# zhexin1904/gtsam_personal

Measured on AMD Instinct MI355X. Metric: LM iterations/sec, higher is better.
Workload: dtype f64; 1 GPU; synthetic BAL 1000 cameras / 100000 points / 1000002 factors (GeneralSFMFactor<Cal3Bundler> + 2 priors), seed 42, METIS ordering (Ordering::Metis of the reference, fixture-carried permutation), LM legacy defaults; ordering=metis, cameras=1000, points=100000, factors=1000002, fronts=100001, parallelism=single GPU

## Files before the change

### gtsam_personal_amd/csrc/kernels_dense.hpp

```cpp
#pragma once
#include <hip/hip_runtime.h>

#include <type_traits>
#include <vector>

#include "kernels_front.hpp"

namespace lmgpu {

typedef double double4_t __attribute__((ext_vector_type(4)));

struct RowSrc {
  int32_t idx;
  int32_t i;
};
inline int32_t append_row_sources(const FrontDesc& F, const std::vector<ChildRef>& childs, const std::vector<int32_t>& cmap, const std::vector<FrontFac>& ffac,
                                  const std::vector<FacDesc>& fd, std::vector<int32_t>& rowptr, std::vector<RowSrc>& rowsrc) {
  std::vector<std::vector<RowSrc>> rows(F.n);
  for (int k = 0; k < F.child_count; k++) {
    const ChildRef& c = childs[F.child_begin + k];
    for (int i = 0; i < c.m; i++) rows[cmap[c.map_begin + i]].push_back(RowSrc{F.child_begin + k, i});
  }
  for (int k = 0; k < F.fac_count; k++) {
    const FrontFac& ff = ffac[F.fac_begin + k];
// ... 35 lines not shown
      const double* J = pool + d.joff;
      const int m = d.rows, nc = d.d0 + d.d1 + d.d2 + 1, p = sr.i;
      for (int q = lane; q < nc; q += 64) {
        const int gq = fac_col(d, ff.c0, ff.c1, ff.c2, q, F.n);
        if (gq > R || (gq == R && q == p)) {
          double v = 0;
          for (int r = 0; r < m; r++) v += J[p * m + r] * J[q * m + r];
          Arow[gq] += v;
        }
      }
    }
    __builtin_amdgcn_fence(__ATOMIC_RELEASE, "wavefront");
    asm volatile("s_waitcnt vmcnt(0)" ::: "memory");
    __builtin_amdgcn_fence(__ATOMIC_ACQUIRE, "wavefront");
  }
}
__global__ __launch_bounds__(256) void hbm_assemble_rows_kernel(FrontDesc F, int64_t f_off, int ld, const int32_t* __restrict__ rowptr,
                                                                const RowSrc* __restrict__ src, const ChildRef* __restrict__ childs,
                                                                const int32_t* __restrict__ cmap, const FrontFac* __restrict__ ffac,
                                                                const FacDesc* __restrict__ fd, double* __restrict__ pool, int with_factors) {
  const int R = blockIdx.x * 4 + (threadIdx.x >> 6);
  if (R >= F.n) return;
  assemble_row_body(F, f_off, ld, rowptr, src, childs, cmap, ffac, fd, pool, R, with_factors != 0);
}

__global__ __launch_bounds__(256) void hbm_damp_kernel(FrontDesc F, int64_t f_off, int ld, const int32_t* __restrict__ fxoff,
                                                        double* __restrict__ pool, double lambda_v, const double* __restrict__ lambda_p, const double* __restrict__ dampw,
                                                        const double* __restrict__ gex) {
  const int i = blockIdx.x * 256 + threadIdx.x;
  if (i >= F.nf) return;
  pool[f_off + (size_t)i * ld + i] += (lambda_p ? *lambda_p : lambda_v) * dampw[fxoff[F.fx_begin + i]];
  if (gex) pool[f_off + (size_t)i * ld + F.n - 1] += gex[fxoff[F.fx_begin + i]];
}

struct ZeroRange {
  int64_t off, count;
};
__global__ __launch_bounds__(256) void zero_ranges_kernel(const ZeroRange* __restrict__ ranges, double* __restrict__ pool) {
  const ZeroRange r = ranges[blockIdx.y];
  double2* p = (double2*)(pool + r.off);
  const int64_t n2 = r.count >> 1;
  for (int64_t i = (int64_t)blockIdx.x * 256 + threadIdx.x; i < n2; i += (int64_t)gridDim.x * 256) p[i] = double2{0.0, 0.0};
}

#define FILL_CHUNK_BYTES 32768
struct FillChunk {
// ... 934 lines not shown
```

### gtsam_personal_amd/csrc/kernels_potrf.hpp

```cpp
#pragma once
#include <hip/hip_runtime.h>

namespace lmgpu {

typedef double double4_t __attribute__((ext_vector_type(4)));

__device__ __forceinline__ double readlane_d(double v, int src_lane) {
  const long long b = __double_as_longlong(v);
  const int lo = __builtin_amdgcn_readlane((int)(b & 0xffffffffLL), src_lane);
  const int hi = __builtin_amdgcn_readlane((int)(b >> 32), src_lane);
  return __longlong_as_double(((long long)hi << 32) | (unsigned int)lo);
}

__device__ __forceinline__ double fast_rsqrt(double p) {
  double y = __builtin_amdgcn_rsq(p);
  const double h = 0.5 * p;
  y = y * fma(-h * y, y, 1.5);
  y = y * fma(-h * y, y, 1.5);
  return y;
}

template <bool INV>
__device__ __forceinline__ bool potrf64_wave_g4(double4_t (&T)[4][4], double4_t (&E)[4], int nrows = 64) {
  const int lane = threadIdx.x & 63, kk = lane >> 4, cc = lane & 15;
// ... 293 lines not shown
          }
        double4_t out = double4_t{0, 0, 0, 0};
#pragma unroll
        for (int sx = 0; sx < 4; sx++) out = __builtin_amdgcn_mfma_f64_16x16x4f64(I16[4 * j + g][4 * sx + kk][cc], acc[sx], out, 0, 0, 0);
        T[g] = out;
        X[j][g] = out;
#pragma unroll
        for (int r = 0; r < 4; r++) {
          const int row = 16 * g + kk + 4 * r;
          if (row < nbj && cvalid) P[(size_t)(64 * j + row) * ld + c0 + cc] = out[r];
        }
      }
    }
  }
}

__global__ __launch_bounds__(256) void panel_trsm_kernel(double* __restrict__ A, int ld, int n, int ko, int kb, const double* __restrict__ inv16) {
  __shared__ double I16[16][16][17];
  panel_trsm_body(A, ld, n, ko, kb, inv16, I16, blockIdx.x);
}

#define TAIL_MAX_M 48
#define TAIL_MAX_KP 256
#define TAIL_LDS_BYTES ((TAIL_MAX_KP * TAIL_MAX_M + TAIL_MAX_M * TAIL_MAX_M + 64 * 65) * 8)
__global__ __launch_bounds__(256) void front_tail_kernel(double* __restrict__ A, int ld, int n, int nf, int p0, int kp, int front_id,
                                                         int* __restrict__ status, double* __restrict__ inv16) {
  extern __shared__ double tsm[];
  const int r0 = p0 + kp, m = n - r0, nft = nf - r0, tid = threadIdx.x;
  double* Pl = tsm;
  double* S = tsm + (size_t)TAIL_MAX_KP * TAIL_MAX_M;
  double(*D)[65] = (double(*)[65])(S + TAIL_MAX_M * TAIL_MAX_M);
  for (int idx = tid; idx < kp * m; idx += 256) {
    const int k = idx / m, j = idx - k * m;
    Pl[idx] = A[(size_t)(p0 + k) * ld + r0 + j];
  }
  for (int idx = tid; idx < m * m; idx += 256) {
    const int i = idx / m, j = idx - i * m;
    S[idx] = (j >= i) ? A[(size_t)(r0 + i) * ld + r0 + j] : 0.0;
  }
  __syncthreads();
  for (int idx = tid; idx < m * m; idx += 256) {
    const int i = idx / m, j = idx - i * m;
    if (j < i) continue;
    double s0 = 0.0, s1 = 0.0;
    int k = 0;
    for (; k + 1 < kp; k += 2) {
      s0 += Pl[k * m + i] * Pl[k * m + j];
      s1 += Pl[(k + 1) * m + i] * Pl[(k + 1) * m + j];
    }
// ... 34 lines not shown
  for (int idx = tid; idx < m * m; idx += 256) {
    const int i = idx / m, j = idx - i * m;
    if (j >= i) A[(size_t)(r0 + i) * ld + r0 + j] = S[idx];
  }
  for (int idx = tid; idx < 64 * 64; idx += 256) {
    const int p = idx >> 6, q = idx & 63;
    D[p][q] = (p < nft && q < nft && q >= p) ? S[p * m + q] : ((p == q) ? 1.0 : 0.0);
  }
  __syncthreads();
  if (tid < 64) {
    const int blk = tid >> 4, c = tid & 15, base = 16 * blk;
    double x[16];
#pragma unroll
    for (int i = 15; i >= 0; i--) {
      double sacc = (i == c) ? 1.0 : 0.0;
#pragma unroll
      for (int kq = i + 1; kq < 16; kq++) sacc -= D[base + i][base + kq] * x[kq];
      x[i] = (i <= c) ? sacc / D[base + i][base + i] : 0.0;
    }
#pragma unroll
    for (int i = 0; i < 16; i++) inv16[(size_t)blk * 256 + i * 16 + c] = x[i];
  }
}

#ifndef PDF_STAMP
#define PDF_STAMP(flags, b, slot)
#endif
#define PDF_TA0 32
#define PDF_MAX_COLTILES 992
#define PDF_PR0 1024
#define PDF_TD0 1536
#define PDF_FLAG_WORDS 8192
#define PDF_MAX_CHAIN_T 114
#define PDF_SPIN_LIMIT 2000000L
#define PDF_LDS_DOUBLES (2 * 64 * DP_LDW)
#define PDF_LDS_BYTES (PDF_LDS_DOUBLES * 8)

__host__ __device__ inline unsigned int pdf_ta_need(int sj) { return sj < 4 ? 4u * (unsigned int)(sj + 1) : 2u; }

__device__ __forceinline__ bool pdf_wait(unsigned int* flags, int w0, unsigned int need0, int w1, unsigned int need1, int* s_ok, int tid) {
  if (tid == 0) {
    bool ok = true;
    for (int q = 0; q < 2 && ok; q++) {
      const int w = q ? w1 : w0;
      const unsigned int need = q ? need1 : need0;
      if (w < 0) continue;
// ... 256 lines not shown
```

### gtsam_personal_amd/csrc/lmgpu.hip

```cpp
#include <hip/hip_runtime.h>
#include <rccl/rccl.h>

#include <algorithm>
#include <chrono>
#include <cmath>
#include <cstdio>
#include <cstdlib>
#include <cstring>
#include <condition_variable>
#include <limits>
#include <mutex>
#include <string>
#include <map>
#include <vector>

#include "../../include/lmgpu.h"
#include "kernels_dense.hpp"
#include "kernels_potrf.hpp"
#include "kernels_step.hpp"
#include "dense_schedule.hpp"
#include "dogleg_step.hpp"
#include "kernels_batched.hpp"
#include "kernels_level.hpp"
#include "kernels_bayes.hpp"
// ... 217 lines not shown
  };
  std::vector<ElimSeg> elim_segs;
  std::vector<int> elim_seg_of;
  bool merge_elim = false;
  FillUpper* d_fill_upper = nullptr;
  int n_fill_upper = 0;
  bool fuse_levels = false;
  LevelTask* d_level_tasks = nullptr;
  LevelSync* d_level_sync = nullptr;
  int n_level_sync = 0;
  int32_t *d_bs_parent = nullptr, *d_bs_pos = nullptr;
  char* d_leafpack = nullptr;
  unsigned int* d_bs_done = nullptr;
  bool use_graph = false;
  int eager_solves = 0;
  hipGraphExec_t solve_graph[2] = {nullptr, nullptr};
  int leaf_group_threads = 256;
  bool no_backsub_groups = false;
  int n_leaf_group_launches = 0;
  bool no_wide16 = false;
  int wide16_max = 256;
  bool bsd_ticket = false;
  bool no_tail = false;
  bool no_chain = false;
  int chain_forms = 0;
  unsigned int* d_pflags = nullptr;
  int pflags_panels = 0;
  unsigned int* bs_flags = nullptr;
  double* pool = nullptr;
  size_t pool_doubles = 0;
  double* vals[2][kNumVarTypes] = {};
  double* saved[kNumVarTypes] = {};
  int cur = 0;
  int32_t* type_xoff[kNumVarTypes] = {};
  double *delta = nullptr, *dampw = nullptr, *hdiag = nullptr, *ebuf0 = nullptr, *ebuf1 = nullptr, *partial = nullptr, *dscal = nullptr,
         *ywork = nullptr;
  int* d_status = nullptr;
  double* h_scal = nullptr;
  int* h_status = nullptr;
  FacDesc* d_fd = nullptr;
  FrontDesc* d_fronts = nullptr;
  FrontFac* d_ffac = nullptr;
  ChildRef* d_childs = nullptr;
  int32_t *d_cmap = nullptr, *d_fxoff = nullptr, *d_sxoff = nullptr, *d_lists = nullptr;
  int32_t *d_hbm_small = nullptr, *d_f_ld = nullptr, *d_med_list = nullptr;
  MedFront* d_med_fronts = nullptr;
  BsdBlock* d_bsd_table = nullptr;
  struct BsdRun {
    int lvl_hi, lvl_lo, begin, count;
  };
  std::vector<BsdRun> bsd_runs;
// ... 323 lines not shown
      h->dampw_is_ones = true;
    }
    return LMGPU_OK;
  }
  int rc = launch_hessian_diag(h);
  if (rc) return rc;
  hipLaunchKernelGGL(clamp_diag_kernel, dim3((h->ntot + 255) / 256), dim3(256), 0, h->stream, h->ntot, (const double*)h->hdiag, h->dampw, min_diag, max_diag);
  h->dampw_is_ones = false;
  return LMGPU_OK;
}

static bool gather_writes(const lmgpu_handle* h, int fi) {
  const lmgpu_handle::GatherRange& G = h->gather[fi];
  if (!(G.write_ok && G.leaf_count > 0 && !h->no_gather_write && h->n_hbm_fronts <= 4)) return false;
  if (h->s_off[fi] < 0) return true;
  return (h->h_fronts[fi].pad & 1) != 0 && (h->comm || h->lgroup);
}

static void add_fill(std::vector<FillChunk>& t, const void* p, size_t bytes, uint32_t value) {
  for (size_t o = 0; o < bytes; o += FILL_CHUNK_BYTES)
    t.push_back(FillChunk{(unsigned long long)(uintptr_t)p + o, (uint32_t)std::min<size_t>(FILL_CHUNK_BYTES, bytes - o), value});
}

static void launch_assemble_rows(lmgpu_handle* h, int fi, int64_t aoff, bool with_factors) {
  const FrontDesc& F = h->h_fronts[fi];
  if (h->row_begin[fi] >= 0 && (F.child_count > 0 || (with_factors && F.fac_count > 0)))
    hipLaunchKernelGGL(hbm_assemble_rows_kernel, dim3((F.n + 3) / 4), dim3(256), 0, h->stream, F, aoff, h->f_ld[fi], (const int32_t*)(h->d_rowptr + h->row_begin[fi]),
                       (const RowSrc*)h->d_rowsrc, (const ChildRef*)h->d_childs, (const int32_t*)h->d_cmap, (const FrontFac*)h->d_ffac,
                       (const FacDesc*)h->d_fd, h->pool, with_factors ? 1 : 0);
}

static void launch_hbm_damp(lmgpu_handle* h, int fi, int64_t aoff, double lambda_v, const double* lambda_p) {
  const FrontDesc& F = h->h_fronts[fi];
  hipLaunchKernelGGL(hbm_damp_kernel, dim3((F.nf + 255) / 256), dim3(256), 0, h->stream, F, aoff, h->f_ld[fi], (const int32_t*)h->d_fxoff, h->pool, lambda_v,
                     lambda_p, (const double*)h->dampw, (const double*)h->gex_active);
}

static int dense_mode_of(const lmgpu_handle* h, int fi) {
  const bool replicated = (h->h_fronts[fi].pad & 1) != 0;
  if (h->s_off[fi] < 0 || !replicated || !(h->comm || h->lgroup)) return DENSE_SINGLE;
  return h->comm ? DENSE_SPLIT_EVENTS : DENSE_SPLIT_HOST;
}

static void chunk_range(int n, int ld, int c, size_t& begin, size_t& count) {
  const int r0c = c * NBO, rows = std::min(n, r0c + NBO) - r0c;
  begin = (size_t)r0c * ld + r0c;
  count = (size_t)rows * ld - r0c;
}

static int wait_chunk(lmgpu_handle* h, double* Asm, int n, int ld, int c) {
  if (h->comm) {
    HIPCHECK(hipStreamWaitEvent(h->stream, h->chunk_ev[c], 0));
// ... 68 lines not shown
      lo = std::min(lo, h->f_off[fi]);
      hi = std::max(hi, h->f_off[fi] + cnt);
    }
  *lo_out = lo;
  *hi_out = hi;
  return n_hbm <= 4 ? HBM_CLEAR_EACH : (hi - lo <= 2 * sum ? HBM_CLEAR_SPAN : HBM_CLEAR_RANGES);
}

static bool backsub_merged(const lmgpu_handle* h) {
  return h->merge_backsub && h->cfg.world_size == 1 && !(h->cfg.flags & LMGPU_FLAG_SPLIT_ROOT);
}

static int ensure_fill_tables(lmgpu_handle* h) {
  int64_t lo, hi;
  const int regime = hbm_clear_regime(h, &lo, &hi);
  if (h->n_fill_elim < 0) {
    std::vector<FillChunk> fills;
    add_fill(fills, h->d_status, sizeof(int), 0x7f7f7f7fu);
    add_fill(fills, h->d_status + 1, sizeof(int), 0u);
    if (h->merge_elim || h->fuse_levels)
      add_fill(fills, h->d_bs_done, (size_t)(h->h_fronts.size() + h->levels.size() + 1) * sizeof(unsigned int), 0u);
    if (h->fuse_levels) add_fill(fills, h->d_level_sync, (size_t)h->n_level_sync * sizeof(LevelSync), 0u);
    if (regime == HBM_CLEAR_SPAN) add_fill(fills, h->pool + lo, (size_t)(hi - lo) * sizeof(double), 0u);
    h->n_fill_elim = (int)fills.size();
    const int rcu = upload(h, &h->d_fill_elim, fills);
    if (rcu) return rcu;
  }
  if (regime == HBM_CLEAR_RANGES && !h->d_zero_ranges) {
    std::vector<ZeroRange> zr;
    for (const LevelWork& L : h->levels)
      for (int fi : L.hbm) {
        const bool gw = gather_writes(h, fi);
        const int64_t cnt = (int64_t)h->h_fronts[fi].n * h->f_ld[fi];
        if (!gw || h->s_off[fi] >= 0) zr.push_back(ZeroRange{h->f_off[fi], cnt});
        if (!gw && h->s_off[fi] >= 0) zr.push_back(ZeroRange{h->s_off[fi], cnt});
      }
    h->n_zero_ranges = (int)zr.size();
    const int rcu = upload(h, &h->d_zero_ranges, zr);
    if (rcu) return rcu;
  }
  if (h->n_fill_backsub < 0) {
    std::vector<FillChunk> fills;
    if (backsub_merged(h)) {
      add_fill(fills, h->d_bs_done, (size_t)(h->h_fronts.size() + h->levels.size() + 1) * sizeof(unsigned int), 0u);
      add_fill(fills, h->delta, h->ntot * sizeof(double), 0xffffffffu);
    }
// ... 117 lines not shown
        ktm = h->kt.begin(LMGPU_KT_SYRK, s);
        hipLaunchKernelGGL(med_syrk_kernel, dim3(4 * S, S, cnt), dim3(256), 0, s, ML, h->pool);
        h->kt.end(ktm, s);
      }
    }
    for (int fi : L.hbm) {
      if (h->is_med[fi]) continue;
      const FrontDesc& F = h->h_fronts[fi];
      const int64_t off = h->f_off[fi];
      const int ld = h->f_ld[fi];
      double* A = h->pool + off;
      const bool own_terms = (F.pad & 2) == 0;
      const lmgpu_handle::GatherRange& G = h->gather[fi];
      const int nchunks = (F.n + NBO - 1) / NBO;
      const int mode = dense_mode_of(h, fi);
      const bool split = mode != DENSE_SINGLE;
      const int64_t aoff = split ? h->s_off[fi] : off;
      double* Asm = h->pool + aoff;

      const int kt = h->kt.begin(LMGPU_KT_HBM_ASSEMBLE, s);
      const bool gwrite = gather_writes(h, fi);
      if (gwrite && G.zero_count > 0)
        hipLaunchKernelGGL(zero_blocks_kernel, dim3(G.zero_count), dim3(128), 0, s, (const GZeroBlock*)(h->d_gzero + G.zero_begin), h->pool, aoff, ld);
      launch_assemble_rows(h, fi, aoff, own_terms && !gwrite);
      if (!gwrite && own_terms) launch_hbm_damp(h, fi, aoff, lambda_v, lambda_p);
      const int schur_masked = dev_switch("LMGPU_SCHUR_UNMASKED") ? 0 : 2;
      if (G.pblk_short > 0)
        hipLaunchKernelGGL((schur_pairs_kernel<1>), dim3((G.pblk_short + 7) & ~7), dim3(64), 0, s, (const GPairBlock*)(h->d_gpblk + G.pblk_begin),
                           (const GPairEntry*)h->d_gpent, h->pool, aoff, ld, G.pblk_short, (gwrite ? 1 : 0) | schur_masked);
      if (G.pblk_long > 0)
        hipLaunchKernelGGL((schur_pairs_kernel<4>), dim3((G.pblk_long + 7) & ~7), dim3(256), 0, s,
                           (const GPairBlock*)(h->d_gpblk + G.pblk_begin + G.pblk_short), (const GPairEntry*)h->d_gpent, h->pool, aoff, ld,
                           G.pblk_long, (gwrite ? 1 : 0) | schur_masked);
#ifdef LMGPU_TEST_HOOKS
      if (h->schur_split_diag) {
        if (G.vblk_count > 0)
          hipLaunchKernelGGL(schur_factor_kernel, dim3(G.vblk_count), dim3(64 * SCHUR_FW), 0, s, (const GVarBlock*)(h->d_gvblk + G.vblk_begin),
                             (const GVarEntry*)h->d_gvent, h->pool, aoff, ld, F.n, schur_masked);
        if (G.leaf_count > 0) {
          double* scal = h->dscal + 4;
          reduce_to(h, h->d_gcorner + G.leaf_begin, G.leaf_count, scal, s, nullptr);
          hipLaunchKernelGGL(add_scalar_kernel, dim3(1), dim3(1), 0, s, Asm + (size_t)(F.n - 1) * ld + F.n - 1, (const double*)scal);
        }
      } else
#endif
      {
        const int vlong = G.vblk_count - G.vblk_short;
        const int corner_short = (G.leaf_count > 0 && vlong == 0) ? 1 : 0, corner_long = (G.leaf_count > 0 && vlong > 0) ? 1 : 0;
        if (G.vblk_short + corner_short > 0)
          hipLaunchKernelGGL((schur_var_kernel<1>), dim3(G.vblk_short + corner_short), dim3(64), 0, s, (const GVarBlock*)(h->d_gvblk + G.vblk_begin),
                             (const GVarEntry*)h->d_gvent, h->pool, aoff, ld, F.n, G.vblk_short, gwrite ? 1 : 0,
                             (const double*)(h->d_gcorner + G.leaf_begin), G.leaf_count);
        if (vlong + corner_long > 0)
          hipLaunchKernelGGL((schur_var_kernel<SCHUR_VAR_WAVES>), dim3(vlong + corner_long), dim3(64 * SCHUR_VAR_WAVES), 0, s,
                             (const GVarBlock*)(h->d_gvblk + G.vblk_begin + G.vblk_short), (const GVarEntry*)h->d_gvent, h->pool, aoff, ld, F.n, vlong,
                             gwrite ? 1 : 0, (const double*)(h->d_gcorner + G.leaf_begin), G.leaf_count);
      }
      if (gwrite && own_terms) {
        if (F.fac_count > 0) launch_assemble_rows(h, fi, aoff, true);
        launch_hbm_damp(h, fi, aoff, lambda_v, lambda_p);
      }
      h->kt.end(kt, s);
      if (mode == DENSE_SPLIT_EVENTS) {
        HIPCHECK(hipEventRecord(h->asm_ev, s));
        HIPCHECK(hipStreamWaitEvent(h->comm_stream, h->asm_ev, 0));
        for (int c = 0; c < nchunks; c++) {
          size_t cb, cn;
          chunk_range(F.n, ld, c, cb, cn);
          NCCLCHECK(ncclAllReduce(Asm + cb, Asm + cb, cn, ncclDouble, ncclSum, h->comm_data ? h->comm_data : h->comm, h->comm_stream));
          HIPCHECK(hipEventRecord(h->chunk_ev[c], h->comm_stream));
        }
      }

      const lmgpu_handle::DensePlan& plan = h->dense_plans[fi];
      h->inv16_owner = fi;
      int kt_run = -1, run_launches = 0;
      double run_flop = 0;
      for (size_t r = 0; r < plan.steps.size(); r++) {
        const DenseStep& st = plan.steps[r];
        const int i = st.i, k0 = i * NBO, kb = std::min(F.nf, k0 + NBO) - k0, r0 = k0 + kb, m = F.n - r0;
        const bool in_run = st.kind == DENSE_STEP_FUSED || (st.kind == DENSE_WAIT_CHUNK && plan.steps[r + 1].kind == DENSE_STEP_FUSED);
        if (!in_run && run_launches > 0) {
          h->kt.end(kt_run, s, run_flop, run_launches);
          run_launches = 0;
          run_flop = 0;
        }
        switch (st.kind) {
          case DENSE_PANEL_DATAFLOW:
          case DENSE_PANEL_TWO_LAUNCH: {
            if (i == 0) HIPCHECK(hipMemsetAsync(h->d_pflags, 0, (size_t)((F.nf + NBO - 1) / NBO + 1) * PDF_FLAG_WORDS * sizeof(unsigned int), s));
            double* inv16 = h->inv16 + (size_t)i * 4096;
            const int ktp = h->kt.begin(LMGPU_KT_PANEL, s);
            if (st.kind == DENSE_PANEL_DATAFLOW) {
              hipLaunchKernelGGL(panel_dataflow_kernel, dim3(kb / 64 + (m + 63) / 64), dim3(256), PDF_LDS_BYTES, s, A, ld, F.n, F.nf, k0, kb, F.id,
                                 h->d_status, inv16, h->d_pflags + (size_t)i * PDF_FLAG_WORDS);
            } else {
              hipLaunchKernelGGL(diag_potrf_kernel, dim3(1), dim3(256), DIAG_LDS_BYTES, s, A, ld, F.nf, k0, kb, F.id, h->d_status, inv16);
              if (m > 0) hipLaunchKernelGGL(panel_trsm_kernel, dim3((m + 63) / 64), dim3(256), 0, s, A, ld, F.n, k0, kb, (const double*)inv16);
            }
            h->kt.end(ktp, s, st.flop);
            break;
          }
          case DENSE_CHAIN: {
            ChainArgs ca{A, ld, F.n, F.nf, i, st.nsteps, F.id, h->d_status, h->inv16, h->d_pflags, h->d_chain_tasks + plan.task_begin[r],
                         split ? (const double*)Asm : nullptr};
#ifdef LMGPU_TEST_HOOKS
            ca.dev_forms = h->chain_forms;
#endif
            const int ktc = h->kt.begin(LMGPU_KT_CHAIN, s);
            hipLaunchKernelGGL(chain_kernel, dim3(plan.task_count[r]), dim3(256), STEP_LDS_BYTES, s, ca);
            h->kt.end(ktc, s, st.flop, 1);
            break;
          }
// ... 5 lines not shown
            a.dev_forms = h->chain_forms;
#endif
            if (run_launches == 0) kt_run = h->kt.begin(LMGPU_KT_SYRK, s);
            hipLaunchKernelGGL(step_kernel, dim3(step_grid(m, kbn)), dim3(256), STEP_LDS_BYTES, s, a);
            run_launches++;
            run_flop += st.flop;
            break;
          }
          case DENSE_UPDATE_QUADRANTS:
          case DENSE_UPDATE_MFMA: {
            const int kts = h->kt.begin(LMGPU_KT_SYRK, s);
            if (st.kind == DENSE_UPDATE_QUADRANTS) {
              const int S = (m + 63) / 64;
              hipLaunchKernelGGL(syrk_quadrants_kernel, dim3(4 * S, S), dim3(256), 0, s, A, ld, F.n, k0, kb, r0);
            } else {
              const int T = (m + 127) / 128;
              hipLaunchKernelGGL(syrk_mfma_kernel, dim3(T, T), dim3(256), kSyrkLds, s, A, ld, F.n, k0, kb, r0, F.n);
            }
            h->kt.end(kts, s, st.flop);
            break;
          }
          case DENSE_TAIL: {
            const int ktt = h->kt.begin(LMGPU_KT_PANEL, s);
            hipLaunchKernelGGL(front_tail_kernel, dim3(1), dim3(256), TAIL_LDS_BYTES, s, A, ld, F.n, F.nf, k0, kb, F.id, h->d_status,
                               h->inv16 + (size_t)(i + 1) * 4096);
            h->kt.end(ktt, s, st.flop);
            break;
          }
          case DENSE_ADD_CHUNK:
          case DENSE_WAIT_CHUNK: {
            const int rcc = st.kind == DENSE_ADD_CHUNK ? add_chunk(h, A, Asm, F.n, ld, st.chunk) : wait_chunk(h, Asm, F.n, ld, st.chunk);
            if (rcc) return rcc;
            break;
          }
        }
      }
      if (run_launches > 0) h->kt.end(kt_run, s, run_flop, run_launches);
    }
  }
  HIPCHECK(hipGetLastError());
  return LMGPU_OK;
}

static int leaf_group_form(const FrontDesc& F, const FrontFac* ffac, const FacDesc* fd, int jcap) {
  if (F.par_ld != -1 || F.pad != 0 || F.nf < 1 || F.nf > LEAFGRP_MAXNF || F.nf > LEAFPACK_MAXNF || F.ld_rsd != F.n) return 0;
  if (F.fac_count < 1 || F.fac_count > LDSF_MAXB) return 0;
  int form = F.nf <= 3 ? 1 : 2;
// ... 98 lines not shown
                         (const int32_t*)h->d_fxoff, (const int32_t*)h->d_sxoff, (const double*)h->pool, h->delta, h->d_bsd_x, h->d_status, 1);
      h->kt.end(kt, s);
    }
    if (L.bsd_count > 0 && brun == -1) {
      const int kt = h->kt.begin(LMGPU_KT_BACKSUB_HBM, s);
      hipLaunchKernelGGL(hbm_backsolve_blocks_kernel, dim3(L.bsd_count), dim3(256), 0, s, (const BsdBlock*)(h->d_bsd_table + L.bsd_begin),
                         (L.bsd_count <= h->num_cus && !h->bsd_ticket) ? (unsigned int*)nullptr : h->d_bsd_ticket + li, (const int32_t*)h->d_fxoff,
                         (const int32_t*)h->d_sxoff, (const double*)h->pool, h->delta, h->d_bsd_x, h->d_status);
      h->kt.end(kt, s);
    }
    for (int fi : L.hbm) {
      const FrontDesc& F = h->h_fronts[fi];
      if (F.nf <= BSS_MAX_NF) continue;
      const int64_t off = h->f_off[fi];
      const int ld = h->f_ld[fi];
      const int kt = h->kt.begin(LMGPU_KT_BACKSUB_HBM, s);
      const bool has_sep = F.n - F.nf - 1 > 0;
      if (has_sep)
        hipLaunchKernelGGL(hbm_rhs_init_kernel, dim3(F.nf), dim3(64), 0, s, F, off, ld, (const int32_t*)h->d_sxoff, (const double*)h->pool,
                           (const double*)h->delta, h->ywork);
      const bool reuse = h->inv16_owner == fi && !dev_switch("LMGPU_NO_INV16_REUSE");
      const bool wide = reuse && !dev_switch("LMGPU_BACKSOLVE_HOP64");
      const int bw = wide ? BSW_NB : NB, nblk = (F.nf + bw - 1) / bw;
      HIPCHECK(hipMemsetAsync(h->bs_flags, 0, (nblk + 1) * sizeof(unsigned int), s));
      HIPCHECK(hipMemsetAsync(h->bs_x, 0xff, (size_t)nblk * bw * sizeof(double), s));
      if (wide) {
        hipLaunchKernelGGL((hbm_backsolve_wide_kernel<false>), dim3(nblk), dim3(512), 0, s, F, off, ld, (const int32_t*)h->d_fxoff, (const double*)h->pool,
                           (const double*)h->inv16, has_sep ? (const double*)h->ywork : (const double*)nullptr, h->bs_x, h->bs_flags, h->delta,
                           h->d_status, h->bs_inv, (unsigned long long*)nullptr);
#ifdef LMGPU_TEST_HOOKS
      } else if (reuse) {
        hipLaunchKernelGGL((hbm_backsolve_dataflow2_kernel<false>), dim3(nblk), dim3(256), 0, s, F, off, ld, (const int32_t*)h->d_fxoff, (const double*)h->pool,
                           (const double*)h->inv16, has_sep ? (const double*)h->ywork : (const double*)nullptr, h->bs_x, h->bs_flags, h->delta,
                           h->d_status, (unsigned long long*)nullptr);
#endif
      } else {
        if (!has_sep)
          hipLaunchKernelGGL(hbm_rhs_init_kernel, dim3(F.nf), dim3(64), 0, s, F, off, ld, (const int32_t*)h->d_sxoff, (const double*)h->pool,
                             (const double*)h->delta, h->ywork);
        hipLaunchKernelGGL((hbm_invert_diag_kernel<NB>), dim3(nblk), dim3(NB), 0, s, (const double*)(h->pool + off), ld, F.nf, h->bs_inv);
        hipLaunchKernelGGL((hbm_backsolve_dataflow_kernel<NB>), dim3(nblk), dim3(256), 0, s, F, off, ld, (const int32_t*)h->d_fxoff,
                           (const double*)h->pool, (const double*)h->bs_inv, (const double*)h->ywork, h->bs_x, h->bs_flags, h->delta,
                           h->d_status);
      }
      h->kt.end(kt, s);
    }
    if (merge) {
      if (L.list_count > 0) {
// ... 261 lines not shown
  HIPCHECK(hipStreamSynchronize(h->stream));
  h->kt.resolve();
  h->solved = true;
  if (h->h_status[1] != 0) {
    h->err = "in-launch dataflow hand-off timed out in front " + std::to_string(h->h_status[1] - 1) + " (spin bound hit)";
    return LMGPU_HIP_ERROR;
  }
  if (*h->h_status < (int)h->h_fronts.size()) {
    const Front& fr = h->plan.fronts[*h->h_status];
    h->failed_slot = fr.vars[0] - h->n_hidden;
    return LMGPU_INDETERMINATE;
  }
  return LMGPU_OK;
}

int do_solve(lmgpu_handle* h, double lambda) {
  const int rc = do_solve_enqueue(h, lambda);
  if (rc) return rc;
  return do_solve_finish(h);
}

int do_retract(lmgpu_handle* h, int from, int to) {
  h->marg_valid = false;
  for (int t = 0; t < kNumVarTypes; t++) {
    const int skip = t == LMGPU_POINT3 ? h->n_hidden : 0;
    const int n = h->plan.type_count[t] - skip;
    if (n == 0) continue;
    hipLaunchKernelGGL(retract_kernel, dim3((n + 255) / 256), dim3(256), 0, h->stream, t, n, (const double*)h->vals[from][t] + 3 * skip,
                       h->vals[to][t] + 3 * skip, (const int32_t*)h->type_xoff[t] + skip, (const double*)h->delta, (const int32_t*)nullptr);
  }
  HIPCHECK(hipGetLastError());
  return LMGPU_OK;
}

void accumulate_times(lmgpu_handle* h, bool with_retract) {
  float ms = 0;
  if (hipEventElapsedTime(&ms, h->ev[1], h->ev[2]) == hipSuccess) h->tim.eliminate_ms += ms;
  if (hipEventElapsedTime(&ms, h->ev[2], h->ev[3]) == hipSuccess) h->tim.backsub_ms += ms;
  if (hipEventElapsedTime(&ms, h->ev[3], h->ev[4]) == hipSuccess) h->tim.linear_error_ms += ms;
  if (with_retract && hipEventElapsedTime(&ms, h->ev[5], h->ev[6]) == hipSuccess) h->tim.retract_error_ms += ms;
}

int enqueue_retract_and_error(lmgpu_handle* h) {
  (void)hipEventRecord(h->ev[5], h->stream);
  const int kt = h->kt.begin(LMGPU_KT_RETRACT_ERROR, h->stream);
  int rc = do_retract(h, h->cur, h->cur ^ 1);
  if (rc) return rc;
  launch_factors<false>(h, h->cur ^ 1);
  reduce_to(h, h->ebuf0, h->n_counted, h->dscal);
  h->kt.end(kt, h->stream);
  rc = allreduce_scalars(h, 0, 1);
  if (rc) return rc;
  (void)hipEventRecord(h->ev[6], h->stream);
// ... 368 lines not shown
    if (rep[fi]) continue;
    h->front_owner[fi] = (fr.parent < 0 || rep[fr.parent]) ? top_owner[fi] : h->front_owner[fr.parent];
  }
  for (int fi = 0; fi < NF; fi++) h->front_active[fi] = rep[fi] || h->front_owner[fi] == R;
}

}

#include "launch_tables.hpp"

extern "C" {

int lmgpu_create(const lmgpu_config* cfg, lmgpu_handle** out) {
  if (!cfg || !out) return LMGPU_INVALID;
  lmgpu_handle* h = new lmgpu_handle();
  h->cfg = *cfg;
  if (h->cfg.world_size < 1) h->cfg.world_size = 1;
  h->device = cfg->device;
  h->two_launch_panel = dev_switch("LMGPU_PANEL_2L") != nullptr;
  h->no_fuse = dev_switch("LMGPU_NO_FUSE") != nullptr;
  h->no_chain = dev_switch("LMGPU_NO_CHAIN") != nullptr;
  h->chain_forms = (dev_switch("LMGPU_CHAIN_FENCED_TILES") ? CHAIN_FORM_FENCED_TILES : 0) | (dev_switch("LMGPU_CHAIN_PREREAD") ? CHAIN_FORM_PREREAD : 0);
  h->no_tail = dev_switch("LMGPU_NO_TAIL") != nullptr;
  h->no_wide16 = dev_switch("LMGPU_NO_WIDE16") != nullptr;
  if (const char* e = dev_switch("LMGPU_LEAF_GROUP_THREADS")) h->leaf_group_threads = atoi(e) == 64 ? 64 : (atoi(e) == 128 ? 128 : 256);
  h->no_backsub_groups = dev_switch("LMGPU_NO_BACKSUB_GROUPS") != nullptr;
  if (const char* e = dev_switch("LMGPU_WIDE16_MAX")) h->wide16_max = atoi(e);
  h->bsd_ticket = dev_switch("LMGPU_BSD_TICKET") != nullptr;
  h->no_gather_write = dev_switch("LMGPU_NO_GATHER_WRITE") != nullptr;
  h->schur_split_diag = dev_switch("LMGPU_SCHUR_SPLIT_DIAG") != nullptr;
  h->pcg_fused = dev_switch("LMGPU_PCG_FUSED") != nullptr;
  if (dev_switch("LMGPU_NO_MERGE")) h->chain_merge = false;
  if (const char* e = dev_switch("LMGPU_CHAIN_SPLIT")) h->chain_split_pct = std::max(0, std::min(100, atoi(e)));
  if (const char* e = dev_switch("LMGPU_CHAIN_FAR")) h->chain_far_pct = std::max(10, std::min(100, atoi(e)));
  *out = h;
  if (h->device >= 0) {
    HIPCHECK(hipSetDevice(h->device));
    {
      hipDeviceProp_t prop;
      HIPCHECK(hipGetDeviceProperties(&prop, h->device));
      h->num_cus = prop.multiProcessorCount;
    }
    HIPCHECK(hipStreamCreate(&h->stream));
    {
      int prio_lo = 0, prio_hi = 0;
      HIPCHECK(hipDeviceGetStreamPriorityRange(&prio_lo, &prio_hi));
      HIPCHECK(hipStreamCreateWithPriority(&h->comm_stream, hipStreamNonBlocking, prio_hi));
    }
    HIPCHECK(hipEventCreateWithFlags(&h->asm_ev, hipEventDisableTiming));
    for (int i = 0; i < 8; i++) HIPCHECK(hipEventCreate(&h->ev[i]));
    HIPCHECK(hipHostMalloc((void**)&h->h_scal, 8 * sizeof(double), hipHostMallocDefault));
    HIPCHECK(hipHostMalloc((void**)&h->h_status, 2 * sizeof(int), hipHostMallocDefault));
    HIPCHECK(hipMalloc((void**)&h->d_lambda, sizeof(double)));
    HIPCHECK(hipMemset(h->d_lambda, 0, sizeof(double)));
    HIPCHECK(hipFuncSetAttribute((const void*)lds_front_kernel<false>, hipFuncAttributeMaxDynamicSharedMemorySize, kLdsLimitN * kLdsLimitN * 8 + kLdsFrontExtra + 64));
    HIPCHECK(hipFuncSetAttribute((const void*)lds_front_kernel<false, 1024>, hipFuncAttributeMaxDynamicSharedMemorySize, kLdsLimitN * kLdsLimitN * 8 + kLdsFrontExtra + 64));
    HIPCHECK(hipFuncSetAttribute((const void*)lds_front_kernel<true>, hipFuncAttributeMaxDynamicSharedMemorySize, kLdsLimitN * kLdsLimitN * 8 + kLdsFrontExtra + 64));
    HIPCHECK(hipFuncSetAttribute((const void*)lds_front_merged_kernel<256>, hipFuncAttributeMaxDynamicSharedMemorySize, kLdsLimitN * kLdsLimitN * 8 + kLdsFrontExtra + 64));
    HIPCHECK(hipFuncSetAttribute((const void*)lds_front_merged_kernel<1024>, hipFuncAttributeMaxDynamicSharedMemorySize, kLdsLimitN * kLdsLimitN * 8 + kLdsFrontExtra + 64));
    HIPCHECK(hipFuncSetAttribute((const void*)level_fused_kernel<256>, hipFuncAttributeMaxDynamicSharedMemorySize, kLdsLimitN * kLdsLimitN * 8 + kLdsFrontExtra + 64));
    HIPCHECK(hipFuncSetAttribute((const void*)level_fused_kernel<1024>, hipFuncAttributeMaxDynamicSharedMemorySize, kLdsLimitN * kLdsLimitN * 8 + kLdsFrontExtra + 64));
    HIPCHECK(hipFuncSetAttribute((const void*)syrk_mfma_kernel, hipFuncAttributeMaxDynamicSharedMemorySize, kSyrkLds));
    HIPCHECK(hipFuncSetAttribute((const void*)lds_backsub_wide_kernel, hipFuncAttributeMaxDynamicSharedMemorySize, (kLdsLimitN * kLdsLimitN + LDSB_TAIL) * 8));
    HIPCHECK(hipFuncSetAttribute((const void*)lds_backsub_merged_kernel, hipFuncAttributeMaxDynamicSharedMemorySize, (kLdsLimitN * kLdsLimitN + LDSB_TAIL) * 8));
    HIPCHECK(hipFuncSetAttribute((const void*)diag_potrf_kernel, hipFuncAttributeMaxDynamicSharedMemorySize, DIAG_LDS_BYTES));
    HIPCHECK(hipFuncSetAttribute((const void*)panel_dataflow_kernel, hipFuncAttributeMaxDynamicSharedMemorySize, PDF_LDS_BYTES));
    HIPCHECK(hipFuncSetAttribute((const void*)step_kernel, hipFuncAttributeMaxDynamicSharedMemorySize, STEP_LDS_BYTES));
    HIPCHECK(hipFuncSetAttribute((const void*)chain_kernel, hipFuncAttributeMaxDynamicSharedMemorySize, STEP_LDS_BYTES));
    HIPCHECK(hipFuncSetAttribute((const void*)front_tail_kernel, hipFuncAttributeMaxDynamicSharedMemorySize, TAIL_LDS_BYTES));
    HIPCHECK(hipFuncSetAttribute((const void*)med_diag_potrf_kernel, hipFuncAttributeMaxDynamicSharedMemorySize, DIAG_LDS_BYTES));
  }
  return LMGPU_OK;
}

int lmgpu_destroy(lmgpu_handle* h) {
  if (!h) return LMGPU_INVALID;
  if (h->device >= 0) {
    (void)hipSetDevice(h->device);
    if (h->stream) (void)hipStreamSynchronize(h->stream);
    if (h->comm_data) ncclCommDestroy(h->comm_data);
    if (h->comm) ncclCommDestroy(h->comm);
    auto fr = [](void* p) {
      if (p) (void)hipFree(p);
    };
    fr(h->pool);
    for (int w = 0; w < 2; w++)
      for (int t = 0; t < kNumVarTypes; t++) fr(h->vals[w][t]);
    for (int t = 0; t < kNumVarTypes; t++) fr(h->type_xoff[t]);
    for (int t = 0; t < kNumVarTypes; t++) fr(h->saved[t]);
    fr(h->gex); fr(h->delta); fr(h->dampw); fr(h->hdiag); fr(h->ebuf0); fr(h->ebuf1); fr(h->partial); fr(h->dscal); fr(h->ywork); fr(h->d_status);
    fr(h->d_fd); fr(h->d_fronts); fr(h->d_ffac); fr(h->d_childs); fr(h->d_cmap); fr(h->d_fxoff); fr(h->d_sxoff); fr(h->d_lists); fr(h->d_hbm_small); fr(h->d_med_list); fr(h->d_med_fronts); fr(h->inv16_med); fr(h->bt_ebuf); fr(h->bt_vec); fr(h->bt_part); fr(h->d_bt_part_off); fr(h->d_bt_ptr); fr(h->d_bt_idx); fr(h->d_f_ld); fr(h->d_f_off);
    fr(h->d_scalar_var); fr(h->d_scalar_col); fr(h->d_vi_ptr); fr(h->d_vi_fac); fr(h->d_vi_pos);
// ... 346 lines not shown
    return LMGPU_INVALID;
  }
  int rc = need_device(h);
  if (rc) return rc;
  for (int t = 0; t < kNumVarTypes; t++) {
    const size_t bytes = std::max<size_t>(1, (size_t)h->plan.type_count[t] * kVarStore[t]) * sizeof(double);
    if (!h->saved[t]) HIPCHECK(hipMalloc((void**)&h->saved[t], bytes));
    HIPCHECK(hipMemcpyAsync(h->saved[t], h->vals[h->cur][t], bytes, hipMemcpyDeviceToDevice, h->stream));
  }
  HIPCHECK(hipStreamSynchronize(h->stream));
  return LMGPU_OK;
}

int lmgpu_restore_values(lmgpu_handle* h) {
  if (!h) return LMGPU_INVALID;
  if (!h->finalized || !h->saved[0]) {
    h->err = "lmgpu_restore_values: refused (!h->finalized || !h->saved[0])";
    return LMGPU_INVALID;
  }
  int rc = need_device(h);
  if (rc) return rc;
  h->marg_valid = false;
  for (int t = 0; t < kNumVarTypes; t++) {
    const size_t bytes = std::max<size_t>(1, (size_t)h->plan.type_count[t] * kVarStore[t]) * sizeof(double);
    HIPCHECK(hipMemcpyAsync(h->vals[h->cur][t], h->saved[t], bytes, hipMemcpyDeviceToDevice, h->stream));
  }
  return LMGPU_OK;
}

int lmgpu_error(lmgpu_handle* h, double* total) {
  if (!h) return LMGPU_INVALID;
  if (!h->finalized || !total || !h->have_values) {
    h->err = "lmgpu_error: refused (!h->finalized || !total || !h->have_values)";
    return LMGPU_INVALID;
  }
  int rc = need_device(h);
  if (rc) return rc;
  if ((rc = need_comm(h))) return rc;
  return compute_error(h, h->cur, total);
}

int lmgpu_linearize(lmgpu_handle* h) {
  if (!h) return LMGPU_INVALID;
  if (!h->finalized || !h->have_values) {
    h->err = "lmgpu_linearize: refused (!h->finalized || !h->have_values)";
    return LMGPU_INVALID;
  }
// ... 1298 lines not shown
```

Baseline: 142.1 LM iterations/s.

## Rewrite front tail with MFMA, fuse damping into assembly, batch retracts and memsets

The front-tail Cholesky kernel is replaced by a register/MFMA version: four waves compute the panel SYRK update, and one wave does a 48-wide partial potrf with inverse 16-blocks. The old LDS scalar version is kept only behind test hooks. The HBM damping kernel is fused into row assembly, per-type retract launches are merged into one multi-type launch, and the pflags/backsolve flag memsets are folded into the existing fill batch when only one front needs them. These changes aim to cut kernel launch count and tail latency, at the cost of more complex numerics and failure checks in the new tail kernel.

Measured after the change: 144.3 LM iterations/s, median of 6. 1.02x the previous value.

```diff
diff --git a/gtsam_personal_amd/csrc/kernels_dense.hpp b/gtsam_personal_amd/csrc/kernels_dense.hpp
--- a/gtsam_personal_amd/csrc/kernels_dense.hpp
+++ b/gtsam_personal_amd/csrc/kernels_dense.hpp
@@ -81,6 +81,21 @@
   const int R = blockIdx.x * 4 + (threadIdx.x >> 6);
   if (R >= F.n) return;
   assemble_row_body(F, f_off, ld, rowptr, src, childs, cmap, ffac, fd, pool, R, with_factors != 0);
+}
+
+__global__ __launch_bounds__(256) void hbm_assemble_rows_damp_kernel(FrontDesc F, int64_t f_off, int ld, const int32_t* __restrict__ rowptr,
+                                                                     const RowSrc* __restrict__ src, const ChildRef* __restrict__ childs,
+                                                                     const int32_t* __restrict__ cmap, const FrontFac* __restrict__ ffac,
+                                                                     const FacDesc* __restrict__ fd, double* __restrict__ pool, int with_factors,
+                                                                     const int32_t* __restrict__ fxoff, double lambda_v, const double* __restrict__ lambda_p,
+                                                                     const double* __restrict__ dampw, const double* __restrict__ gex) {
+  const int R = blockIdx.x * 4 + (threadIdx.x >> 6);
+  if (R >= F.n) return;
+  assemble_row_body(F, f_off, ld, rowptr, src, childs, cmap, ffac, fd, pool, R, with_factors != 0);
+  if (R < F.nf && (threadIdx.x & 63) == 0) {
+    pool[f_off + (size_t)R * ld + R] += (lambda_p ? *lambda_p : lambda_v) * dampw[fxoff[F.fx_begin + R]];
+    if (gex) pool[f_off + (size_t)R * ld + F.n - 1] += gex[fxoff[F.fx_begin + R]];
+  }
 }
 
 __global__ __launch_bounds__(256) void hbm_damp_kernel(FrontDesc F, int64_t f_off, int ld, const int32_t* __restrict__ fxoff,
diff --git a/gtsam_personal_amd/csrc/kernels_potrf.hpp b/gtsam_personal_amd/csrc/kernels_potrf.hpp
--- a/gtsam_personal_amd/csrc/kernels_potrf.hpp
+++ b/gtsam_personal_amd/csrc/kernels_potrf.hpp
@@ -339,9 +339,199 @@
 
 #define TAIL_MAX_M 48
 #define TAIL_MAX_KP 256
-#define TAIL_LDS_BYTES ((TAIL_MAX_KP * TAIL_MAX_M + TAIL_MAX_M * TAIL_MAX_M + 64 * 65) * 8)
+
+__device__ __forceinline__ bool potrf48_partial_wave(double4_t (&T)[3][3], double4_t (&E)[3], int nft) {
+  const int lane = threadIdx.x & 63, kk = lane >> 4, cc = lane & 15;
+  bool failed = false;
+#pragma unroll
+  for (int g = 0; g < 3; g++) {
+#pragma unroll
+    for (int r = 0; r < 4; r++) E[g][r] = (kk + 4 * r == cc) ? 1.0 : 0.0;
+    if (16 * g >= nft) continue;
+#pragma unroll
+    for (int q = 0; q < 4; q++) {
+      if (16 * g + 4 * q >= nft) continue;
+      const int na = min(4, nft - 16 * g - 4 * q);
+      double m[4][4];
+#pragma unroll
+      for (int a = 0; a < 4; a++)
+#pragma unroll
+        for (int b = a; b < 4; b++) m[a][b] = readlane_d(T[g][g][q], 16 * a + 4 * q + b);
+      double R[4][4], inv[4];
+#pragma unroll
+      for (int a = 0; a < 4; a++) {
+        const bool act = a < na;
+        double p = m[a][a];
+#pragma unroll
+        for (int k = 0; k < a; k++) p -= R[k][a] * R[k][a];
+        failed |= act && (p <= 0.0);
+        p = (p > 0.0) ? p : ((p == p && p != 0.0) ? fabs(p) : 1.0);
+        p = act ? p : 1.0;
+        const double rs = fast_rsqrt(p);
+        inv[a] = rs;
+        R[a][a] = p * rs;
+#pragma unroll
+        for (int b = a + 1; b < 4; b++) {
+          double v = m[a][b];
+#pragma unroll
+          for (int k = 0; k < a; k++) v -= R[k][a] * R[k][b];
+          R[a][b] = act ? v * rs : 0.0;
+        }
+      }
+      double W[4][4];
+#pragma unroll
+      for (int a = 0; a < 4; a++) {
+        W[a][a] = inv[a];
+#pragma unroll
+        for (int b = a + 1; b < 4; b++) {
+          double v = 0;
+#pragma unroll
+          for (int k = a; k < b; k++) v += W[a][k] * R[k][b];
+          W[a][b] = -v * inv[b];
+        }
+      }
+      double aop = 0.0;
+#pragma unroll
+      for (int k = 0; k < 4; k++)
+#pragma unroll
+        for (int i = k; i < 4; i++) aop = (kk == k && cc == i) ? W[k][i] : aop;
+      const double aop_e = (kk != cc && cc >= na) ? 0.0 : aop;
+      double bop = 0.0, bop_e = 0.0;
+      {
+        const double4_t x = __builtin_amdgcn_mfma_f64_16x16x4f64(aop, T[g][g][q], double4_t{0, 0, 0, 0}, 0, 0, 0);
+        T[g][g][q] = x[0];
+        if (q < 3) {
+          bop = (cc >= 4 * (q + 1) && kk < na) ? -T[g][g][q] : 0.0;
+          bop_e = (16 * g + cc < nft) ? bop : 0.0;
+          T[g][g] = __builtin_amdgcn_mfma_f64_16x16x4f64(bop, T[g][g][q], T[g][g], 0, 0, 0);
+        }
+      }
+#pragma unroll
+      for (int h = g + 1; h < 3; h++) {
+        const double4_t x = __builtin_amdgcn_mfma_f64_16x16x4f64(aop, T[g][h][q], double4_t{0, 0, 0, 0}, 0, 0, 0);
+        T[g][h][q] = x[0];
+        if (q < 3) T[g][h] = __builtin_amdgcn_mfma_f64_16x16x4f64(bop, T[g][h][q], T[g][h], 0, 0, 0);
+      }
+      {
+        const double4_t x = __builtin_amdgcn_mfma_f64_16x16x4f64(aop_e, E[g][q], double4_t{0, 0, 0, 0}, 0, 0, 0);
+        E[g][q] = x[0];
+        if (q < 3) E[g] = __builtin_amdgcn_mfma_f64_16x16x4f64(bop_e, E[g][q], E[g], 0, 0, 0);
+      }
+    }
+#pragma unroll
+    for (int g2 = g + 1; g2 < 3; g2++)
+#pragma unroll
+      for (int h = g2; h < 3; h++)
+#pragma unroll
+        for (int s = 0; s < 4; s++) {
+          const double aneg = (16 * g + 4 * s + kk < nft) ? -T[g][g2][s] : 0.0;
+          T[g2][h] = __builtin_amdgcn_mfma_f64_16x16x4f64(aneg, T[g][h][s], T[g2][h], 0, 0, 0);
+        }
+  }
+  return failed;
+}
+
 __global__ __launch_bounds__(256) void front_tail_kernel(double* __restrict__ A, int ld, int n, int nf, int p0, int kp, int front_id,
                                                          int* __restrict__ status, double* __restrict__ inv16) {
+  __shared__ double part[3][24][64];
+  const int r0 = p0 + kp, m = n - r0, nft = nf - r0;
+  const int wave = threadIdx.x >> 6, lane = threadIdx.x & 63, kk = lane >> 4, cc = lane & 15;
+  const double* P = A + (size_t)p0 * ld + r0;
+  double pv[16][3];
+#pragma unroll
+  for (int s = 0; s < 16; s++)
+#pragma unroll
+    for (int t = 0; t < 3; t++) {
+      const int row = 64 * wave + 4 * s + kk, col = 16 * t + cc;
+      const double v = P[(size_t)min(row, kp - 1) * ld + min(col, m - 1)];
+      pv[s][t] = (row < kp && col < m) ? v : 0.0;
+    }
+  double4_t T[3][3];
+  double* C = A + (size_t)r0 * ld + r0;
+  if (wave == 0) {
+#pragma unroll
+    for (int g = 0; g < 3; g++)
+#pragma unroll
+      for (int h = g; h < 3; h++)
+#pragma unroll
+        for (int r = 0; r < 4; r++) {
+          const int row = 16 * g + kk + 4 * r, col = 16 * h + cc;
+          const double v = C[(size_t)min(row, m - 1) * ld + min(col, m - 1)];
+          T[g][h][r] = (row < m && col < m && col >= row) ? v : 0.0;
+        }
+  }
+  double4_t acc[6];
+#pragma unroll
+  for (int x = 0; x < 6; x++) acc[x] = double4_t{0, 0, 0, 0};
+#pragma unroll
+  for (int s = 0; s < 16; s++) {
+    int x = 0;
+#pragma unroll
+    for (int ti = 0; ti < 3; ti++)
+#pragma unroll
+      for (int tj = ti; tj < 3; tj++, x++) acc[x] = __builtin_amdgcn_mfma_f64_16x16x4f64(pv[s][ti], pv[s][tj], acc[x], 0, 0, 0);
+  }
+  if (wave > 0) {
+#pragma unroll
+    for (int x = 0; x < 6; x++)
+#pragma unroll
+      for (int r = 0; r < 4; r++) part[wave - 1][4 * x + r][lane] = acc[x][r];
+  }
+  __syncthreads();
+  if (wave > 0) return;
+  {
+    int x = 0;
+#pragma unroll
+    for (int g = 0; g < 3; g++)
+#pragma unroll
+      for (int h = g; h < 3; h++, x++)
+#pragma unroll
+        for (int r = 0; r < 4; r++)
+          T[g][h][r] -= ((acc[x][r] + part[0][4 * x + r][lane]) + part[1][4 * x + r][lane]) + part[2][4 * x + r][lane];
+  }
+  double4_t E[3];
+  bool failed = potrf48_partial_wave(T, E, nft);
+  {
+    const int p1 = nft - 1, p2 = max(nft - 2, 0);
+    double v1 = 0.0, v2 = 0.0;
+#pragma unroll
+    for (int g = 0; g < 3; g++)
+#pragma unroll
+      for (int r = 0; r < 4; r++) {
+        v1 = ((p1 >> 4) == g && ((p1 & 15) >> 2) == r) ? T[g][g][r] : v1;
+        v2 = ((p2 >> 4) == g && ((p2 & 15) >> 2) == r) ? T[g][g][r] : v2;
+      }
+    const double r1 = __shfl(v1, 16 * (p1 & 3) + (p1 & 15), 64);
+    if (nft >= 2) {
+      const double r2 = __shfl(v2, 16 * (p2 & 3) + (p2 & 15), 64);
+      if (!(frexp_exp_d(r2) - frexp_exp_d(r1) < 12)) failed = true;
+    } else if (nf >= 2) {
+      if (!(frexp_exp_d(A[(size_t)(nf - 2) * ld + nf - 2]) - frexp_exp_d(r1) < 12)) failed = true;
+    } else if (!(frexp_exp_d(r1) > -12)) {
+      failed = true;
+    }
+  }
+  if (failed && lane == 0) atomicMin(status, front_id);
+#pragma unroll
+  for (int g = 0; g < 3; g++)
+#pragma unroll
+    for (int r = 0; r < 4; r++) {
+      const int row = 16 * g + kk + 4 * r;
+#pragma unroll
+      for (int h = g; h < 3; h++) {
+        const int col = 16 * h + cc;
+        if (row < m && col < m && col >= row) C[(size_t)row * ld + col] = T[g][h][r];
+      }
+      inv16[(size_t)g * 256 + cc * 16 + kk + 4 * r] = E[g][r];
+    }
+#pragma unroll
+  for (int r = 0; r < 4; r++) inv16[(size_t)3 * 256 + cc * 16 + kk + 4 * r] = (kk + 4 * r == cc) ? 1.0 : 0.0;
+}
+
+#ifdef LMGPU_TEST_HOOKS
+#define TAIL_LDS_BYTES ((TAIL_MAX_KP * TAIL_MAX_M + TAIL_MAX_M * TAIL_MAX_M + 64 * 65) * 8)
+__global__ __launch_bounds__(256) void front_tail_scalar_kernel(double* __restrict__ A, int ld, int n, int nf, int p0, int kp, int front_id,
+                                                                int* __restrict__ status, double* __restrict__ inv16) {
   extern __shared__ double tsm[];
   const int r0 = p0 + kp, m = n - r0, nft = nf - r0, tid = threadIdx.x;
   double* Pl = tsm;
@@ -422,6 +612,7 @@
     for (int i = 0; i < 16; i++) inv16[(size_t)blk * 256 + i * 16 + c] = x[i];
   }
 }
+#endif
 
 #ifndef PDF_STAMP
 #define PDF_STAMP(flags, b, slot)
diff --git a/gtsam_personal_amd/csrc/lmgpu.hip b/gtsam_personal_amd/csrc/lmgpu.hip
--- a/gtsam_personal_amd/csrc/lmgpu.hip
+++ b/gtsam_personal_amd/csrc/lmgpu.hip
@@ -263,11 +263,13 @@
   int wide16_max = 256;
   bool bsd_ticket = false;
   bool no_tail = false;
+  bool tail_scalar = false;
   bool no_chain = false;
   int chain_forms = 0;
   unsigned int* d_pflags = nullptr;
   int pflags_panels = 0;
   unsigned int* bs_flags = nullptr;
+  bool pflags_prefilled = false, bs_prefilled = false;
   double* pool = nullptr;
   size_t pool_doubles = 0;
   double* vals[2][kNumVarTypes] = {};
@@ -637,12 +639,20 @@
     t.push_back(FillChunk{(unsigned long long)(uintptr_t)p + o, (uint32_t)std::min<size_t>(FILL_CHUNK_BYTES, bytes - o), value});
 }
 
-static void launch_assemble_rows(lmgpu_handle* h, int fi, int64_t aoff, bool with_factors) {
+static bool launch_assemble_rows(lmgpu_handle* h, int fi, int64_t aoff, bool with_factors, bool damp = false, double lambda_v = 0.0,
+                                 const double* lambda_p = nullptr) {
   const FrontDesc& F = h->h_fronts[fi];
-  if (h->row_begin[fi] >= 0 && (F.child_count > 0 || (with_factors && F.fac_count > 0)))
+  if (!(h->row_begin[fi] >= 0 && (F.child_count > 0 || (with_factors && F.fac_count > 0)))) return false;
+  if (damp)
+    hipLaunchKernelGGL(hbm_assemble_rows_damp_kernel, dim3((F.n + 3) / 4), dim3(256), 0, h->stream, F, aoff, h->f_ld[fi],
+                       (const int32_t*)(h->d_rowptr + h->row_begin[fi]), (const RowSrc*)h->d_rowsrc, (const ChildRef*)h->d_childs, (const int32_t*)h->d_cmap,
+                       (const FrontFac*)h->d_ffac, (const FacDesc*)h->d_fd, h->pool, with_factors ? 1 : 0, (const int32_t*)h->d_fxoff, lambda_v, lambda_p,
+                       (const double*)h->dampw, (const double*)h->gex_active);
+  else
     hipLaunchKernelGGL(hbm_assemble_rows_kernel, dim3((F.n + 3) / 4), dim3(256), 0, h->stream, F, aoff, h->f_ld[fi], (const int32_t*)(h->d_rowptr + h->row_begin[fi]),
                        (const RowSrc*)h->d_rowsrc, (const ChildRef*)h->d_childs, (const int32_t*)h->d_cmap, (const FrontFac*)h->d_ffac,
                        (const FacDesc*)h->d_fd, h->pool, with_factors ? 1 : 0);
+  return true;
 }
 
 static void launch_hbm_damp(lmgpu_handle* h, int fi, int64_t aoff, double lambda_v, const double* lambda_p) {
@@ -757,6 +767,21 @@
       add_fill(fills, h->d_bs_done, (size_t)(h->h_fronts.size() + h->levels.size() + 1) * sizeof(unsigned int), 0u);
     if (h->fuse_levels) add_fill(fills, h->d_level_sync, (size_t)h->n_level_sync * sizeof(LevelSync), 0u);
     if (regime == HBM_CLEAR_SPAN) add_fill(fills, h->pool + lo, (size_t)(hi - lo) * sizeof(double), 0u);
+    int n_plan = 0, n_wide = 0, plan_fi = -1, wide_fi = -1;
+    for (const LevelWork& L : h->levels)
+      for (int fi : L.hbm) {
+        if (!h->is_med[fi]) n_plan++, plan_fi = fi;
+        if (h->h_fronts[fi].nf > BSS_MAX_NF) n_wide++, wide_fi = fi;
+      }
+    h->pflags_prefilled = n_plan == 1;
+    h->bs_prefilled = n_wide == 1;
+    if (h->pflags_prefilled)
+      add_fill(fills, h->d_pflags, (size_t)((h->h_fronts[plan_fi].nf + NBO - 1) / NBO + 1) * PDF_FLAG_WORDS * sizeof(unsigned int), 0u);
+    if (h->bs_prefilled) {
+      const int nf = h->h_fronts[wide_fi].nf;
+      add_fill(fills, h->bs_flags, (size_t)((nf + NB - 1) / NB + 1) * sizeof(unsigned int), 0u);
+      add_fill(fills, h->bs_x, (size_t)((nf + BSW_NB - 1) / BSW_NB) * BSW_NB * sizeof(double), 0xffffffffu);
+    }
     h->n_fill_elim = (int)fills.size();
     const int rcu = upload(h, &h->d_fill_elim, fills);
     if (rcu) return rcu;
@@ -920,8 +945,8 @@
       const bool gwrite = gather_writes(h, fi);
       if (gwrite && G.zero_count > 0)
         hipLaunchKernelGGL(zero_blocks_kernel, dim3(G.zero_count), dim3(128), 0, s, (const GZeroBlock*)(h->d_gzero + G.zero_begin), h->pool, aoff, ld);
-      launch_assemble_rows(h, fi, aoff, own_terms && !gwrite);
-      if (!gwrite && own_terms) launch_hbm_damp(h, fi, aoff, lambda_v, lambda_p);
+      const bool damp_here = !gwrite && own_terms;
+      if (!launch_assemble_rows(h, fi, aoff, own_terms && !gwrite, damp_here, lambda_v, lambda_p) && damp_here) launch_hbm_damp(h, fi, aoff, lambda_v, lambda_p);
       const int schur_masked = dev_switch("LMGPU_SCHUR_UNMASKED") ? 0 : 2;
       if (G.pblk_short > 0)
         hipLaunchKernelGGL((schur_pairs_kernel<1>), dim3((G.pblk_short + 7) & ~7), dim3(64), 0, s, (const GPairBlock*)(h->d_gpblk + G.pblk_begin),
@@ -955,8 +980,7 @@
                              gwrite ? 1 : 0, (const double*)(h->d_gcorner + G.leaf_begin), G.leaf_count);
       }
       if (gwrite && own_terms) {
-        if (F.fac_count > 0) launch_assemble_rows(h, fi, aoff, true);
-        launch_hbm_damp(h, fi, aoff, lambda_v, lambda_p);
+        if (!(F.fac_count > 0 && launch_assemble_rows(h, fi, aoff, true, true, lambda_v, lambda_p))) launch_hbm_damp(h, fi, aoff, lambda_v, lambda_p);
       }
       h->kt.end(kt, s);
       if (mode == DENSE_SPLIT_EVENTS) {
@@ -986,7 +1010,7 @@
         switch (st.kind) {
           case DENSE_PANEL_DATAFLOW:
           case DENSE_PANEL_TWO_LAUNCH: {
-            if (i == 0) HIPCHECK(hipMemsetAsync(h->d_pflags, 0, (size_t)((F.nf + NBO - 1) / NBO + 1) * PDF_FLAG_WORDS * sizeof(unsigned int), s));
+            if (i == 0 && !h->pflags_prefilled) HIPCHECK(hipMemsetAsync(h->d_pflags, 0, (size_t)((F.nf + NBO - 1) / NBO + 1) * PDF_FLAG_WORDS * sizeof(unsigned int), s));
             double* inv16 = h->inv16 + (size_t)i * 4096;
             const int ktp = h->kt.begin(LMGPU_KT_PANEL, s);
             if (st.kind == DENSE_PANEL_DATAFLOW) {
@@ -1038,7 +1062,13 @@
           }
           case DENSE_TAIL: {
             const int ktt = h->kt.begin(LMGPU_KT_PANEL, s);
-            hipLaunchKernelGGL(front_tail_kernel, dim3(1), dim3(256), TAIL_LDS_BYTES, s, A, ld, F.n, F.nf, k0, kb, F.id, h->d_status,
+#ifdef LMGPU_TEST_HOOKS
+            if (h->tail_scalar)
+              hipLaunchKernelGGL(front_tail_scalar_kernel, dim3(1), dim3(256), TAIL_LDS_BYTES, s, A, ld, F.n, F.nf, k0, kb, F.id, h->d_status,
+                                 h->inv16 + (size_t)(i + 1) * 4096);
+            else
+#endif
+            hipLaunchKernelGGL(front_tail_kernel, dim3(1), dim3(256), 0, s, A, ld, F.n, F.nf, k0, kb, F.id, h->d_status,
                                h->inv16 + (size_t)(i + 1) * 4096);
             h->kt.end(ktt, s, st.flop);
             break;
@@ -1183,8 +1213,10 @@
       const bool reuse = h->inv16_owner == fi && !dev_switch("LMGPU_NO_INV16_REUSE");
       const bool wide = reuse && !dev_switch("LMGPU_BACKSOLVE_HOP64");
       const int bw = wide ? BSW_NB : NB, nblk = (F.nf + bw - 1) / bw;
-      HIPCHECK(hipMemsetAsync(h->bs_flags, 0, (nblk + 1) * sizeof(unsigned int), s));
-      HIPCHECK(hipMemsetAsync(h->bs_x, 0xff, (size_t)nblk * bw * sizeof(double), s));
+      if (!h->bs_prefilled) {
+        HIPCHECK(hipMemsetAsync(h->bs_flags, 0, (nblk + 1) * sizeof(unsigned int), s));
+        HIPCHECK(hipMemsetAsync(h->bs_x, 0xff, (size_t)nblk * bw * sizeof(double), s));
+      }
       if (wide) {
         hipLaunchKernelGGL((hbm_backsolve_wide_kernel<false>), dim3(nblk), dim3(512), 0, s, F, off, ld, (const int32_t*)h->d_fxoff, (const double*)h->pool,
                            (const double*)h->inv16, has_sep ? (const double*)h->ywork : (const double*)nullptr, h->bs_x, h->bs_flags, h->delta,
@@ -1492,13 +1524,23 @@
 
 int do_retract(lmgpu_handle* h, int from, int to) {
   h->marg_valid = false;
+  static_assert(kNumVarTypes <= 7, "RetractMulti holds seven entries");
+  RetractMulti rm{};
+  int ne = 0, maxn = 0;
   for (int t = 0; t < kNumVarTypes; t++) {
     const int skip = t == LMGPU_POINT3 ? h->n_hidden : 0;
     const int n = h->plan.type_count[t] - skip;
     if (n == 0) continue;
-    hipLaunchKernelGGL(retract_kernel, dim3((n + 255) / 256), dim3(256), 0, h->stream, t, n, (const double*)h->vals[from][t] + 3 * skip,
-                       h->vals[to][t] + 3 * skip, (const int32_t*)h->type_xoff[t] + skip, (const double*)h->delta, (const int32_t*)nullptr);
-  }
+    rm.type[ne] = t;
+    rm.n[ne] = n;
+    rm.cur[ne] = (const double*)h->vals[from][t] + 3 * skip;
+    rm.out[ne] = h->vals[to][t] + 3 * skip;
+    rm.xoff[ne] = (const int32_t*)h->type_xoff[t] + skip;
+    rm.sel[ne] = nullptr;
+    maxn = std::max(maxn, n);
+    ne++;
+  }
+  if (ne > 0) hipLaunchKernelGGL(retract_multi_kernel, dim3((maxn + 255) / 256, ne), dim3(256), 0, h->stream, rm, (const double*)h->delta);
   HIPCHECK(hipGetLastError());
   return LMGPU_OK;
 }
@@ -1913,6 +1955,7 @@
   h->no_chain = dev_switch("LMGPU_NO_CHAIN") != nullptr;
   h->chain_forms = (dev_switch("LMGPU_CHAIN_FENCED_TILES") ? CHAIN_FORM_FENCED_TILES : 0) | (dev_switch("LMGPU_CHAIN_PREREAD") ? CHAIN_FORM_PREREAD : 0);
   h->no_tail = dev_switch("LMGPU_NO_TAIL") != nullptr;
+  h->tail_scalar = dev_switch("LMGPU_TAIL_SCALAR") != nullptr;
   h->no_wide16 = dev_switch("LMGPU_NO_WIDE16") != nullptr;
   if (const char* e = dev_switch("LMGPU_LEAF_GROUP_THREADS")) h->leaf_group_threads = atoi(e) == 64 ? 64 : (atoi(e) == 128 ? 128 : 256);
   h->no_backsub_groups = dev_switch("LMGPU_NO_BACKSUB_GROUPS") != nullptr;
@@ -1958,7 +2001,9 @@
     HIPCHECK(hipFuncSetAttribute((const void*)panel_dataflow_kernel, hipFuncAttributeMaxDynamicSharedMemorySize, PDF_LDS_BYTES));
     HIPCHECK(hipFuncSetAttribute((const void*)step_kernel, hipFuncAttributeMaxDynamicSharedMemorySize, STEP_LDS_BYTES));
     HIPCHECK(hipFuncSetAttribute((const void*)chain_kernel, hipFuncAttributeMaxDynamicSharedMemorySize, STEP_LDS_BYTES));
-    HIPCHECK(hipFuncSetAttribute((const void*)front_tail_kernel, hipFuncAttributeMaxDynamicSharedMemorySize, TAIL_LDS_BYTES));
+#ifdef LMGPU_TEST_HOOKS
+    HIPCHECK(hipFuncSetAttribute((const void*)front_tail_scalar_kernel, hipFuncAttributeMaxDynamicSharedMemorySize, TAIL_LDS_BYTES));
+#endif
     HIPCHECK(hipFuncSetAttribute((const void*)med_diag_potrf_kernel, hipFuncAttributeMaxDynamicSharedMemorySize, DIAG_LDS_BYTES));
   }
   return LMGPU_OK;
@@ -2351,7 +2396,8 @@
   if (rc) return rc;
   h->marg_valid = false;
   for (int t = 0; t < kNumVarTypes; t++) {
-    const size_t bytes = std::max<size_t>(1, (size_t)h->plan.type_count[t] * kVarStore[t]) * sizeof(double);
+    if (h->plan.type_count[t] == 0) continue;
+    const size_t bytes = (size_t)h->plan.type_count[t] * kVarStore[t] * sizeof(double);
     HIPCHECK(hipMemcpyAsync(h->vals[h->cur][t], h->saved[t], bytes, hipMemcpyDeviceToDevice, h->stream));
   }
   return LMGPU_OK;
```
